# limuhit/360-Image-Compression

Hardware: AMD Instinct MI355X
Metric: ERP Mpixels/s enc+dec @512x1024 model-idx 3; bitstream bit-exact vs ref (higher is better)
Workload: dtype f32; 1 GPU; 192/GPU synthetic 512x1024 ERPs, model-idx 3 --ssim seed, latent+importance bitstreams, entropy enc+dec; streams=3, masks=smooth

## Files before the change

### 360-image-compression_amd/csrc/cconv4_kernels.hip

```cpp
#include "common.h"
#include "conv_plan.h"

#include "cconv_tree.h"
#include "need.h"

#define C4_COLS 68
#define C4_WSLOTS 128

static inline bool conv4_ok(const lic360_conv_plan *p) {
    return p->ksz == 5 && (p->cin == 1 || p->cin == 4) && p->cout >= 1 && p->cout <= 4 && p->ngroup <= 64;
}

__global__ void k_conv4_pack(const float *__restrict__ weight, float *__restrict__ quads, int wblk, int nb, int ngroup, int cin, int cout, int hidden) {
    const long per_net = (long)ngroup * ngroup * C4_WSLOTS * 4, total = per_net * nb;
    const int C = ngroup * cin, nout = ngroup * cout;
    for (long i = (long)blockIdx.x * blockDim.x + threadIdx.x; i < total; i += (long)gridDim.x * blockDim.x) {
        int r = (int)(i & 3), leaf = (int)((i >> 2) & 31), c = (int)((i >> 7) & 3);
        long t = i / (C4_WSLOTS * 4);
        int tc = (int)(t % ngroup), g = (int)((t / ngroup) % ngroup), b = (int)(t / ((long)ngroup * ngroup));
        int tap = cin == 4 ? leaf : c + 4 * leaf, gid = cin == 4 ? ((c - tap) & 3) : 0;
        float v = 0.0f;
        if (tap < 25 && r < cout) {
            int kh = tap / 5, kw = tap % 5;
            int L = g + 4 - kh - kw + hidden;
            if (L > ngroup) L = ngroup;
            if (tc < L) v = weight[(((long)b * nout + g * cout + r) * C + tc * cin + gid) * 25 + tap];
        }
        const long qb = (long)(b * ngroup + g) * wblk;
        const int ln = (leaf & 15) * 4 + r;
        if (cin == 4) quads[(qb + (tc >> 1)) * 1024 + c * 256 + ln * 4 + (tc & 1) * 2 + (leaf >> 4)] = v;
        else if (leaf < 16) quads[(qb + (tc >> 2)) * 1024 + c * 256 + ln * 4 + (tc & 3)] = v;
    }
}

LIC360_API int lic360_conv4_supported(const lic360_conv_plan *p) { return p && conv4_ok(p) ? 1 : 0; }
static inline long conv4_slot_floats(const lic360_conv_plan *p) { return (long)p->ngroup * p->ngroup * C4_WSLOTS * 4; }
static inline int conv4_wblk(const lic360_conv_plan *p) { return p->cin == 4 ? (p->ngroup + 1) / 2 : 2 * ((p->ngroup + 7) / 8); }
static inline long conv4_quad_floats(const lic360_conv_plan *p) { return (long)p->ngroup * conv4_wblk(p) * 1024; }
LIC360_API long lic360_conv4_packed_floats(const lic360_conv_plan *p) {
    return p && conv4_ok(p) ? conv4_quad_floats(p) : 0;
}
LIC360_API int lic360_conv4_pack(void *stream, const lic360_conv_plan *p, const float *weight, int nb, float *packed) {
    ARG_CHECK(p && conv4_ok(p) && weight && packed && nb > 0);
    const long total = conv4_slot_floats(p) * nb;
    HIP_TRY(hipMemsetAsync(packed, 0, (size_t)conv4_quad_floats(p) * nb * sizeof(float), (hipStream_t)stream));
    hipLaunchKernelGGL(k_conv4_pack, dim3(lic360_blocks(total, 4)), dim3(256), 0, (hipStream_t)stream, weight, packed, conv4_wblk(p), nb, p->ngroup,
                       p->cin, p->cout, p->constrain == 5 ? 0 : 1);
    LAUNCH_CHECK();
    return 0;
}

#define C4_PS 3
#define C4_THREADS (C4_PS * 4 * 64)
#define C4_COMB_FLOATS (C4_PS * 4 * 4 * 64)

#include "cconv4v6_dc.inc"

int lic360_cconv4_dc_plane_mode(void *stream, const lic360_conv_plan *p, const float *x, const float *packed4, const float *bias,
                                const float *act, const float *residual, float *out, int n, int h, int w, int nb, int psum, int x_mod, int mode) {
    ARG_CHECK(p && conv4_ok(p) && x && packed4 && bias && out && n > 0 && nb > 0 && n % nb == 0 && x_mod > 0 && x_mod <= n);
    if (psum < 0 || psum >= h + w + p->ngroup - 2) return 0;
    return launch_cconv4v6_dc((hipStream_t)stream, p, x, packed4, bias, act, residual, out, n, h, w, nb, psum, x_mod, (mode & 2) != 0,
                              (mode >> 2) & 3);
}
int lic360_cconv4_dc_plane_list(void *stream, const lic360_conv_plan *p, const float *x, const float *packed4, const float *bias,
                                const float *act, const float *residual, float *out, int n, int h, int w, int nb, int psum, int x_mod,
                                const void *list, const int *cnt, int cap) {
    ARG_CHECK(p && conv4_ok(p) && x && packed4 && bias && out && n > 0 && nb > 0 && n % nb == 0 && x_mod > 0 && x_mod <= n);
    if (psum < 0 || psum >= h + w + p->ngroup - 2) return 0;
    return launch_cconv4v6_dc_list((hipStream_t)stream, p, x, packed4, bias, act, residual, out, n, h, w, nb, psum, x_mod, (const uint4 *)list, cnt, cap);
}
int lic360_dc4_env_mode(void) {
    const char *gsm = getenv("LIC360_DC_GSTEP");
    return (getenv("LIC360_NOPACK") ? 2 : 0) | (gsm && gsm[0] == '1' ? 4 : (gsm && gsm[0] == '3' ? 8 : 0));
}
LIC360_API int lic360_cconv4_dc_plane(void *stream, const lic360_conv_plan *p, const float *x, const float *packed4, const float *bias,
                                      const float *act, const float *residual, float *out, int n, int h, int w, int nb, int psum, int x_mod) {
    static const int mode = lic360_dc4_env_mode();
    return lic360_cconv4_dc_plane_mode(stream, p, x, packed4, bias, act, residual, out, n, h, w, nb, psum, x_mod, mode);
}

#define C4_TAIL_FLOATS 4096
LIC360_API long lic360_conv4_buffer_floats(int layout, long planes, int h, int w) {
    if (planes <= 0 || h <= 0 || w <= 0 || layout != 0) return 0;
    return planes * ((long)D3_SP(h, w) * D3_HP(h)) + C4_TAIL_FLOATS;
}
LIC360_API int lic360_dc4_layout(int h, int w, int *rows, int *pitch, int *row0, int *col0) {
    ARG_CHECK(rows && pitch && row0 && col0 && h > 0 && w > 0);
    *rows = D3_SP(h, w); *pitch = D3_HP(h); *row0 = D3_S0; *col0 = D3_C0;
    return 0;
}
```

### 360-image-compression_amd/csrc/cconv4v6_dc.inc

```
#define D6_GRID 256
#define D6_TAPE_BLOCKS 16
#define D6_TAPE_WAVES 6
#define D3_S0 (4 + C4_PS - 1)
#define D3_C0 2
#define D3_SP(h, w) ((h) + (w) - 1 + 2 * D3_S0)
#define D3_HP(h) ((h) + 2 * D3_C0)
struct Dc3Args {
    const float *x, *packed, *bias, *act, *residual;
    float *out;
    int ngroup, cout, hidden, H, W, npb, x_mod, N, psum, n_gb, n_gbv, nseg, pack0, gstep;
    int wblk;
    int nprod;
    int tape_c, tape_n, tape_total;
    unsigned tape_magic;
    unsigned tape_nw4[2];
};
struct Dc3Packed {
    const float *x, *packed, *bias, *act, *residual;
    float *out;
    unsigned w0;
    unsigned hw;
    int npb, x_mod, N;
    unsigned pg;
    int wblk, tape_n, tape_total;
// ... 85 lines not shown
__device__ __forceinline__ void conv6_diags(f32x4 *acc, const float *r0, float w0, float w1) {
    static_for<9>([&](auto dd) {
        constexpr int d = decltype(dd)::value, kmin = d > 4 ? d - 4 : 0, kmax = d < 4 ? d : 4;
        if constexpr (d >= D_LO && d <= D_HI && (CIN == 4 || (d & 3) == CLS)) {
            static_for<kmax - kmin + 1>([&](auto kk) {
                constexpr int kh = kmin + decltype(kk)::value, tap = 5 * kh + (d - kh), i = CIN == 4 ? tap : (tap - CLS) / 4;
                acc[i] = mfma4<i % 16>(i < 16 ? w0 : w1, r0[d], acc[i]);
            });
        }
    });
    __builtin_amdgcn_sched_barrier(0);
}
template <int CIN, int CLS>
__device__ __forceinline__ void conv6_align(f32x4 *acc) {
    static_for<9>([&](auto dd) {
        constexpr int d = decltype(dd)::value, kmin = d > 4 ? d - 4 : 0, kmax = d < 4 ? d : 4;
        constexpr int k0 = kmax < 2 ? kmax : (kmin > 2 ? kmin : 2);
        if constexpr (CIN == 4 || (d & 3) == CLS) {
            static_for<kmax - kmin + 1>([&](auto kk) {
                constexpr int kh = kmin + decltype(kk)::value, tap = 5 * kh + (d - kh), i = CIN == 4 ? tap : (tap - CLS) / 4, sh = kh - k0;
                static_for<(sh > 0 ? sh : -sh)>([&](auto) {
#pragma unroll
                    for (int r = 0; r < 4; ++r) acc[i][r] = sh > 0 ? dpp_shl1(acc[i][r]) : dpp_shr1(acc[i][r]);
                });
            });
        }
    });
}

struct W8 {
    float a0, a1, a2, a3, b0, b1, b2, b3;
    template <int H, int J> __device__ __forceinline__ float get() const {
        if constexpr (H == 0) return J == 0 ? a0 : (J == 1 ? a1 : (J == 2 ? a2 : a3));
        else return J == 0 ? b0 : (J == 1 ? b1 : (J == 2 ? b2 : b3));
    }
};

#define D6_SEG_STEP 60
#define D6_NSEG(h) ((h) <= 64 ? 1 : 1 + ((h) - 62 + D6_SEG_STEP - 1) / D6_SEG_STEP)
#ifdef DC6_STAMP
__device__ unsigned long long dc6_stamps[256 * 12 * 10];
#ifndef DC6_STAMP_CIN
#define DC6_STAMP_CIN 4
#endif
#define DC6_T(i) do { if constexpr (CIN == DC6_STAMP_CIN && !SEG) { const unsigned long long t_ = __builtin_amdgcn_s_memtime(); st[i] += t_ - t0; t0 = t_; } } while (0)
LIC360_API int lic360_dc6_stamps(unsigned long long *host_out, int clear) {
    if (host_out) HIP_TRY(hipMemcpyFromSymbol(host_out, HIP_SYMBOL(dc6_stamps), sizeof(dc6_stamps)));
    if (clear) { static unsigned long long z[256 * 12 * 10]; HIP_TRY(hipMemcpyToSymbol(HIP_SYMBOL(dc6_stamps), z, sizeof(z))); }
    return 0;
}
#else
#define DC6_T(i)
#endif
template <int CIN, int CLS, bool SEG, bool LAT = false, bool TAPE = false, bool LIST = false>
__device__ __forceinline__ void dc6_body(const Dc3Args &a, const Dc3Tape *tape, const uint4 *__restrict__ list, const int *__restrict__ lcnt, float *xs, float *comb,
                                         int (*trec)[16], int tid, int lane, int ps) {
    static_assert(!LIST || (TAPE && !SEG && !LAT), "list launches are throughput-mode launches of images of at most 64 rows");
    constexpr int XQ = D6_XQ(CIN), XFL = D6_XFL(CIN);
    static_assert(XQ <= C4_THREADS, "one quad slot per thread");
    constexpr int XPLANE = D6_ROWS * D6_COLS;
    const int H = a.H, W = a.W, G = a.ngroup, S = H + W - 1, HP = D3_HP(H);
    const int gs = a.gstep;
    constexpr int TCS = CIN == 1 ? 4 : 1;
    const long SKP = (long)D3_SP(H, W) * HP, tcs = 4 * SKP;
    f32x4 acc[NAcc<CIN>::value];
#ifdef DC6_STAMP
    unsigned long long st[10] = {0, 0, 0, 0, 0, 0, 0, 0, 0, 0}, t0 = __builtin_amdgcn_s_memtime();
    const unsigned long long t_entry = t0;
#endif
    const bool flat = gs == 1;
    const int xcd = flat ? 0 : blockIdx.x & 7, xstep = flat ? 1 : 8, wg_in_xcd = flat ? blockIdx.x : blockIdx.x >> 3;
    const int wgs_per_xcd = flat ? D6_GRID : (D6_GRID - xcd + 7) >> 3;
    auto nth_task = [&](int k) __attribute__((always_inline)) { return k * wgs_per_xcd + ((k & 1) ? wgs_per_xcd - 1 - wg_in_xcd : wg_in_xcd); };
    const int ns_x = flat ? a.N : (a.N - xcd + 7) >> 3;
    const int nseg = SEG ? a.nseg : 1;
    constexpr bool PACK = true;
    const bool pack_last = PACK && SEG && a.pack0 != 0;
    const int per_j = SEG ? ns_x * (nseg - 1) + (pack_last ? (ns_x + 1) >> 1 : ns_x) : 0;
    const int tape_c = TAPE ? a.tape_c : 0;
    const unsigned nw4[2] = {a.tape_nw4[0], a.tape_nw4[1]};
    auto blk_tasks = [&](int j) __attribute__((always_inline)) {
        return tape_c ? a.tape_n * (int)((nw4[(j >> 3) & 1] >> ((j & 7) * 4)) & 15u) : ns_x;
    };
    uint4 lrec = make_uint4(0u, 0u, 0u, 0u);
    if constexpr (LIST) {
        if (CLS == 0 && ps == 0) {
            int u = nth_task(lane);
            if (u > a.tape_total - 1) u = a.tape_total - 1;
            lrec = list[(long)xcd * a.tape_total + u];
        }
    }
    int n_my_ = 0;
    if constexpr (LIST) n_my_ = __builtin_amdgcn_readfirstlane(lcnt[xcd]);
    else if constexpr (SEG) n_my_ = per_j * a.n_gbv;
    else if (tape_c) n_my_ = a.tape_total;
    else n_my_ = ns_x * a.n_gbv;
    const int n_my = n_my_;
    int pk = -1, pq = 0;
    auto decode = [&](int u, int &g0, int &n, int &s0, int &seg, int &nb2, int &prb, int &packed) __attribute__((always_inline)) {
        nb2 = -1; prb = 0; packed = 0;
        if constexpr (LIST) {
            uint4 r;
            if (pk < 64) {
                r.x = (unsigned)__builtin_amdgcn_readlane((int)lrec.x, pk); r.y = (unsigned)__builtin_amdgcn_readlane((int)lrec.y, pk);
                r.z = (unsigned)__builtin_amdgcn_readlane((int)lrec.z, pk); r.w = (unsigned)__builtin_amdgcn_readlane((int)lrec.w, pk);
            } else r = list[(long)xcd * a.tape_total + u];
            g0 = (int)(r.x & 127u);
            n = (int)(r.x >> 10);
            s0 = a.psum - g0;
            seg = 0;
            if ((r.x >> 7) & 7u) { seg = (int)(r.y & 0x3fffffu); nb2 = (int)r.z; prb = (int)r.w; packed = 4; }
            packed |= (int)((r.y >> 22) & 7u) << 4;
        } else if constexpr (!SEG) {
            int j = 0, rem = u;
            for (; j < a.n_gbv - 1 && rem >= blk_tasks(j); ++j) rem -= blk_tasks(j);
            g0 = (a.n_gb - 1 - j) * gs;
            s0 = a.psum - g0;
            seg = 0;
// ... 100 lines not shown
                }
                t_off = cov ? offA + sh : 0u;
                t_off0 = cov ? offA0 + sh : 0u;
            } else if (SEG && PACK && ipacked) {
                const bool hb = qc > 8;
                const unsigned shift = hb ? (unsigned)(((long)((inb >= 0 ? inb : n) % a.x_mod) - (long)(n % a.x_mod)) * G * CIN * SKP * 4 - 9 * 16) : 0u;
                t_off = offA + shift;
                t_off0 = offA0 + shift;
            } else {
                const int lo = is0 - (gs - 1) - W + 1 - irb, hi = (is0 < H - 1 ? is0 : H - 1) - irb;
                const bool col_ok = qc >= ((lo > 0 ? lo : 0) >> 2) && qc <= ((hi + 4) >> 2);
                t_off = col_ok ? offA : 0u;
                t_off0 = col_ok ? offA0 : 0u;
            }
        }
        const int gg = ig0 + ps < G ? ig0 + ps : G - 1;
        iwp = (const char *)(a.packed + (((long)(n / a.npb) * G + gg) * a.wblk) * 1024);
    };
    if (!ivalid) return;
    issue_setup();
    const long tcs_b = tcs * 4;
    constexpr int WPSTEP = CIN == 4 ? 4096 : 8192;
    const char *px = ixn, *pw = iwp;
    auto issue_x2 = [&](f32x4 &ra, f32x4 &rb, int &tc0) __attribute__((always_inline)) -> const char * {
        const char *pwr = pw;
        tc0 = itc;
        unsigned oa, ob;
        if constexpr (CIN == 4) {
            oa = rowA < irl - itc ? t_off : t_off0;
            ob = rowA < irl - itc - 1 ? t_off : t_off0;
        } else {
            const int ta = itc + tcoA, tb = ta + TCS;
            oa = rowA < irl - ta ? t_off : t_off0;
            ob = rowA < irl - tb ? t_off : t_off0;
            if (ta >= G) oa = offP0;
            if (tb >= G) ob = offP0;
        }
        ra = *(const f32x4 *)(px + oa);
        rb = *(const f32x4 *)(px + (itc + TCS < G ? tcs_b : 0) + ob);
        if (ivalid) {
            px += 2 * tcs_b;
            pw += WPSTEP;
            itc += 2 * TCS;
            if (itc >= iL) {
                itc = 0;
                ++iq;
                ivalid = rec(iq, 0) != 0;
                if (ivalid) { issue_setup(); px = ixn; pw = iwp; }
                else { px -= 2 * tcs_b; pw -= WPSTEP; itc = tc0; }
            }
        }
        return pwr;
    };
    auto issue_w2 = [&](const char *p, int tc0, W8 &w) __attribute__((always_inline)) {
        (void)tc0;
        const f32x4 v = *(const f32x4 *)(p + offW);
        w.a0 = v[0]; w.a1 = v[1];
        if constexpr (CIN == 4) { w.b0 = v[2]; w.b1 = v[3]; }
        else {
            const f32x4 u = *(const f32x4 *)(p + offW + 4096);
            w.a2 = v[2]; w.a3 = v[3];
            w.b0 = u[0]; w.b1 = u[1]; w.b2 = u[2]; w.b3 = u[3];
        }
    };
    constexpr bool MIDST = D6_STAGE_AT_END == 0 || CIN == 1 || LAT || LIST;
    constexpr int NB = D6_NB, NBUF = 2 * D6_NB;
    static_assert(NB == 1 || NB == 2, "one or two double steps per barrier");
    f32x4 xa0 = {0.f, 0.f, 0.f, 0.f}, xb0 = xa0, xa1 = xa0, xb1 = xa0;
    W8 w0, w1;
    int tcw;
    { const char *p = issue_x2(xa0, xb0, tcw); issue_w2(p, tcw, w0); }
    { const char *p = issue_x2(xa1, xb1, tcw); issue_w2(p, tcw, w1); }
    if (hasA) { *(f32x4 *)ldsA = xa0; *(f32x4 *)(ldsA + XFL) = xb0; }
    int tcw_next, tcw_next2 = 0;
    const char *pw_next = issue_x2(xa0, xb0, tcw_next), *pw_next2 = nullptr;
    if constexpr (NB == 2) {
        if (hasA) { *(f32x4 *)(ldsA + 2 * XFL) = xa1; *(f32x4 *)(ldsA + 3 * XFL) = xb1; }
        pw_next2 = issue_x2(xa1, xb1, tcw_next2);
    }
    const f32x4 zero4 = {0.f, 0.f, 0.f, 0.f};
    int tq = 0, tc = 0, g0 = 0, n = 0, Lwg = 0, g = 0, s = 0, step = 0;
    bool glive = false, lane_ok = false;
    int n_lane = 0;
    float e_bias = 0.f, e_act = 0.f, e_res = 0.f;
    long e_oi = 0;
    const float *const act_p = a.act ? a.act : a.bias, *const res_p = a.residual ? a.residual : a.x;
    const float *const xl0 = xs + (C4_PS - 1 - ps) * D6_COLS + lane;
    auto task_setup = [&]() __attribute__((always_inline)) {
        g0 = rec(tq, 1); n = rec(tq, 2);
        const int s0 = rec(tq, 3), seg = rec(tq, 4), nb2 = rec(tq, 5), prb = rec(tq, 6);
        const int pk7 = rec(tq, 7), packed = pk7 & 15;
        Lwg = steps_of(g0);
        g = g0 + ps;
        s = s0 - ps;
        const int rb = packed == 4 ? 0 : ((SEG && !packed) ? D6_SEG_STEP * seg : prb);
        int row = rb + lane;
        n_lane = n;
        bool half_ok = true;
        if (TAPE && packed == 4) {
            half_ok = false;
            row = 0;
#pragma unroll
            for (int wi = 0; wi < 3; ++wi) {
                const unsigned wd = (unsigned)(wi == 0 ? seg : (wi == 1 ? nb2 : prb));
                const int k = wd & 7, slo = (wd >> 3) & 63, shi = (wd >> 9) & 63, a0 = (wd >> 15) & 63;
                if ((wd >> 21) != 0 && lane >= a0 && lane <= a0 + (shi - slo)) { half_ok = true; row = slo + lane - a0; n_lane = n + 8 * k; }
            }
        } else if (SEG && PACK && packed) {
            if (lane >= 36) { row = rb + lane - 36; n_lane = nb2 >= 0 ? nb2 : n; half_ok = nb2 >= 0; }
            else half_ok = lane < 28;
        }
        int sc;
        {
            int lo = s >= W ? s - W + 1 : 0, hi = s < H ? s : H - 1;
            const int segx = packed == 4 ? 0 : seg;
            if (lo < seg_lo(segx)) lo = seg_lo(segx);
            if (hi > seg_hi(segx)) hi = seg_hi(segx);
            glive = g < G && ps < gs && s >= 0 && s < S && lo <= hi && ((pk7 >> (4 + ps)) & 1) != 0;
            lane_ok = glive && half_ok && row >= lo && row <= hi;
            sc = s < 0 ? 0 : (s >= S ? S - 1 : s);
        }
#pragma unroll
        for (int i = 0; i < NAcc<CIN>::value; ++i) acc[i] = zero4;
        tc = 0;
        const int nout = G * a.cout, gc = g < G ? g : G - 1;
        const int o = gc * a.cout + (CLS < a.cout ? CLS : a.cout - 1), bid = (n / a.npb) * nout + o;
        e_oi = ((long)n_lane * nout + o) * SKP + (long)(sc + D3_S0) * HP + row + D3_C0;
        e_bias = a.bias[bid];
        e_act = act_p[bid];
        e_res = res_p[a.residual ? e_oi : 0];
    };
    auto epilogue = [&]() __attribute__((always_inline)) {
        conv6_align<CIN, CLS>(acc);
        const f32x4 part = tree4_eval<CIN, CLS>(acc);
        float *const cb = CIN == 1 ? comb + (tq & 1) * C4_COMB_FLOATS : comb;
#pragma unroll
        for (int r = 0; r < 4; ++r) cb[((ps * 4 + CLS) * 4 + r) * 64 + lane] = part[r];
        __syncthreads();
        const int r = CLS;
        if (lane_ok && r < a.cout) {
            const float f0 = cb[((ps * 4 + 0) * 4 + r) * 64 + lane], f1 = cb[((ps * 4 + 1) * 4 + r) * 64 + lane];
            const float f2 = cb[((ps * 4 + 2) * 4 + r) * 64 + lane], f3 = cb[((ps * 4 + 3) * 4 + r) * 64 + lane];
            float sv = ((f0 + f2) + (f1 + f3)) + e_bias;
            if (a.act) { if (sv < 0) sv = sv * e_act; }
            if (a.residual) sv = sv + e_res;
            a.out[e_oi] = sv;
        }
    };
    task_setup();
#define DC6_SUB(H_, J_, W_)                                                                     \
    if constexpr ((J_) < TCS) {                                                                 \
        constexpr int k = (H_) * TCS + (J_);                                                    \
        const int dl = dlim - k;                     \
        if (dl > 0 && tc + k < Lwg) {                                                           \
            float r0[9];                                                                        \
            conv6_load<CIN, CLS, XPLANE>(r0, xl + (H_) * XFL + (J_) * XPLANE);                  \
            __builtin_amdgcn_sched_barrier(0);                                                  \
            const float wa = W_.template get<(H_), (CIN == 4 ? 0 : (J_))>(), wb = W_.template get<(H_), 1>(); \
            conv6_diags<CIN, CLS, 0, 3>(acc, r0, wa, wb);                                       \
            if (dl > 4) conv6_diags<CIN, CLS, 4, 5>(acc, r0, wa, wb);                           \
            if (dl > 6) conv6_diags<CIN, CLS, 6, 8>(acc, r0, wa, wb);                           \
        }                                                                                       \
    }
#define DC6_HALF(H_, W_) DC6_SUB(H_, 0, W_) DC6_SUB(H_, 1, W_) DC6_SUB(H_, 2, W_) DC6_SUB(H_, 3, W_)
#define D6_STAGE_WRITE(XA_, XB_)                                                                \
        if (hasA) {                                                                             \
            float *q = ldsA + ((step + NB) & (NBUF - 1)) * (2 * XFL);                           \
            *(f32x4 *)q = XA_;                                                                  \
            *(f32x4 *)(q + XFL) = XB_;                                                          \
        }
#define D6_STAGE_BLOCK(XA_, XB_)                                                                \
        D6_STAGE_WRITE(XA_, XB_)                                                                \
        DC6_T(8);                        \
        pw_new = issue_x2(XA_, XB_, tcw_new);                                                   \
        __builtin_amdgcn_sched_barrier(0);
#define D6_STAGE_MID(XA_, XB_) if constexpr (MIDST) { D6_STAGE_BLOCK(XA_, XB_) }
#define D6_STAGE_END(XA_, XB_) if constexpr (!MIDST) { D6_STAGE_BLOCK(XA_, XB_) }
#define DC6_SUBSTEP(XA_, XB_, W_)                                                               \
    {                                                                                           \
        if (tc >= Lwg) {                                                                        \
            epilogue();                                                                         \
            ++tq;                                                                               \
            if (producer) produce();               \
            if (rec(tq, 0)) task_setup();                                                       \
            else { done = true; glive = false; Lwg = 0x7fffffff; }                              \
            DC6_ST7                                                                             \
        }                                                                                       \
        DC6_T(0);                                                                               \
        if (NB == 1 || (step & 1) == 0) __syncthreads();                                        \
        DC6_T(1);                                                                               \
        const int dlim = glive ? g + 4 + a.hidden - tc : 0;                                     \
        const float *xl = xl0 + (step & (NBUF - 1)) * (2 * XFL);                                \
        int tcw_new = 0;                                                                        \
        const char *pw_new = nullptr;                                                           \
        DC6_HALF(0, W_)                                                                         \
        DC6_T(2);                                                                               \
        D6_STAGE_MID(XA_, XB_)                                                                  \
        DC6_T(3);                                                                               \
        DC6_HALF(1, W_)                                                                         \
        D6_STAGE_END(XA_, XB_)                                                                  \
        DC6_T(4);                                                                               \
        issue_w2(pw_next, tcw_next, W_);                                                        \
        if constexpr (NB == 2) { pw_next = pw_next2; tcw_next = tcw_next2; pw_next2 = pw_new; tcw_next2 = tcw_new; } \
        else { pw_next = pw_new; tcw_next = tcw_new; }                                          \
        tc += 2 * TCS;                                                                          \
        ++step;                                                                                 \
        DC6_T(5);                                                                               \
        DC6_ST6                                                                                 \
    }
#ifdef DC6_STAMP
#define DC6_ST6 st[6] += 1;
#define DC6_ST7 st[7] += 1;
#else
#define DC6_ST6
#define DC6_ST7
#endif
    bool done = false;
    do {
        if constexpr (NB == 2) {
            DC6_SUBSTEP(xa0, xb0, w0)
            DC6_SUBSTEP(xa1, xb1, w1)
        } else {
            DC6_SUBSTEP(xa1, xb1, w0)
            DC6_SUBSTEP(xa0, xb0, w1)
        }
    } while (!done);
#ifdef DC6_STAMP
    if constexpr (CIN == DC6_STAMP_CIN && !SEG) {
        st[9] = __builtin_amdgcn_s_memtime() - t_entry;
        if (lane == 0) for (int i = 0; i < 10; ++i) dc6_stamps[((blockIdx.x & 255) * 12 + ps * 4 + CLS) * 10 + i] += st[i];
    }
#endif
#undef DC6_ST6
#undef DC6_ST7
#undef DC6_HALF
#undef DC6_SUB
#undef DC6_SUBSTEP
}

template <int CIN, bool SEG, bool LAT, bool TAPE, bool LIST = false>
__device__ __forceinline__ void dc6_kernel(const Dc3Packed &p, const Dc3Tape *tape, const uint4 *list = nullptr, const int *lcnt = nullptr) {
    __shared__ float xs[4 * D6_NB * D6_XFL(CIN)];
    __shared__ float comb[2 * C4_COMB_FLOATS];
    __shared__ int trec[8][16];
    const Dc3Args a = dc6_unpack(p);
    const int tid = threadIdx.x, lane = tid & 63;
    const int wave = __builtin_amdgcn_readfirstlane(tid >> 6), ps = wave >> 2, cls = wave & 3;
    switch (cls) {
        case 0: dc6_body<CIN, 0, SEG, LAT, TAPE, LIST>(a, tape, list, lcnt, xs, comb, trec, tid, lane, ps); break;
        case 1: dc6_body<CIN, 1, SEG, LAT, TAPE, LIST>(a, tape, list, lcnt, xs, comb, trec, tid, lane, ps); break;
        case 2: dc6_body<CIN, 2, SEG, LAT, TAPE, LIST>(a, tape, list, lcnt, xs, comb, trec, tid, lane, ps); break;
        default: dc6_body<CIN, 3, SEG, LAT, TAPE, LIST>(a, tape, list, lcnt, xs, comb, trec, tid, lane, ps); break;
    }
}
template <int CIN, bool SEG, bool LAT = false>
__global__ __launch_bounds__(C4_THREADS) void k_cconv4v6(Dc3Packed p) { dc6_kernel<CIN, SEG, LAT, false>(p, nullptr); }
template <int CIN>
__global__ __launch_bounds__(C4_THREADS) void k_cconv4v6t(Dc3Packed p, Dc3Tape tape) { dc6_kernel<CIN, false, false, true>(p, &tape); }
template <int CIN>
__global__ __launch_bounds__(C4_THREADS) void k_cconv4v6l(Dc3Packed p, const uint4 *list, const int *lcnt) { dc6_kernel<CIN, false, false, true, true>(p, nullptr, list, lcnt); }

static void dc6_build_tape(Dc3Args &a, Dc3Tape &tape, int h, int w, int cin, int n, int gs, bool nopack) {
    a.tape_c = 0; a.tape_n = 1; a.tape_total = 0; a.tape_magic = 0u; a.tape_nw4[0] = a.tape_nw4[1] = 0u;
    for (int j = 0; j < D6_TAPE_BLOCKS; ++j) tape.s[j] = 0u;
    const int S = h + w - 1, m = a.npb / 8;
    int c = 0;
    for (int t = D6_TAPE_WAVES; t >= 2 && !c; --t) if (m % t == 0) c = t;
    const bool ok = !nopack && a.nseg == 1 && gs == C4_PS && n % 8 == 0 && a.npb % 8 == 0 && c >= 2 && a.x_mod % (8 * c) == 0 && a.n_gbv <= D6_TAPE_BLOCKS &&
                    8.0 * c * a.ngroup * cin * (double)D3_SP(h, w) * D3_HP(h) * 4.0 < 4294967296.0;
    if (!ok) return;
    long old_tasks = 0, new_tasks = 0;
    int nws[D6_TAPE_BLOCKS];
    for (int j = 0; j < a.n_gbv; ++j) {
        const int gb = a.n_gb - 1 - j, s0 = a.psum - gb * C4_PS;
        int lo = 1 << 30, hi = -1;
        for (int q = 0; q < C4_PS; ++q) {
            const int sq = s0 - q;
            if (gb * C4_PS + q >= a.ngroup || sq < 0 || sq >= S) continue;
            const int l = sq >= w ? sq - w + 1 : 0, u = sq < h ? sq : h - 1;
            if (l < lo) lo = l;
            if (u > hi) hi = u;
        }
        int nw = 0, k = 0, slo = lo;
        unsigned starts = 0u;
        bool fits = hi >= 0;
        while (fits && k < c) {
            if (nw >= D6_TAPE_WAVES) { fits = false; break; }
            if (nw & 1) starts |= ((unsigned)k | (unsigned)slo << 3) << (9 * (nw >> 1));
            unsigned pc[3];
            if (dc6_wave_pieces(lo, hi, h, c, k, slo, pc) == 0) fits = false;
            ++nw;
        }
        if (!fits || nw >= c) {
            nw = c;
            starts = 0u;
        }
        tape.s[j] = starts;
        a.tape_nw4[j >> 3] |= (unsigned)nw << ((j & 7) * 4);
        nws[j] = nw;
        new_tasks += (long)nw * (m / c);
        old_tasks += m;
    }
    if (new_tasks > 0 && new_tasks < old_tasks) {
        a.tape_c = c;
        a.tape_n = n / 8 / c;
        a.tape_magic = (unsigned)((4294967296ull + a.tape_n - 1) / a.tape_n);
        for (int j = 0; j < a.n_gbv; ++j) a.tape_total += a.tape_n * nws[j];
    }
}

static bool dc6_schedule(Dc3Args &a, Dc3Tape &tape, int ngroup, int cin, int cout, int constrain, int n, int h, int w, int nb, int psum, int x_mod, bool nopack, int gstep_mode) {
    a.ngroup = ngroup; a.cout = cout; a.hidden = constrain == 5 ? 0 : 1; a.H = h; a.W = w; a.npb = n / nb; a.x_mod = x_mod; a.N = n;
    a.psum = psum;
    const int S = h + w - 1;
    int gb_lo = 1 << 30, gb_hi = -1;
    const int n_gb3 = (ngroup + C4_PS - 1) / C4_PS;
    const int gs = gstep_mode == 1 || (gstep_mode == 0 && (long)n * n_gb3 <= 128 && D6_NSEG(h) == 1) ? 1 : C4_PS;
    a.gstep = gs;
    {
        const int tcs2 = cin == 4 ? 2 : 8, lmin0 = (gs - 1) + 4 + a.hidden, lmin = lmin0 < ngroup ? lmin0 : ngroup;
        const int dmin = (lmin + tcs2 - 1) / tcs2, lead = (4 + dmin - 1) / dmin;
        a.nprod = lead + 2 < 6 ? lead + 2 : 6;
    }
    const int n_gb_all = (ngroup + gs - 1) / gs;
    for (int gb = 0; gb < n_gb_all; ++gb) {
        int s0 = psum - gb * gs;
        if (s0 - (gs - 1) >= S || s0 < 0) continue;
        if (gb < gb_lo) gb_lo = gb;
        if (gb > gb_hi) gb_hi = gb;
    }
    a.tape_c = 0; a.pack0 = 0;
    if (gb_hi < 0) return false;
    a.n_gb = gb_hi + 1;
    a.n_gbv = gb_hi - gb_lo + 1;
    a.nseg = D6_NSEG(h);
    dc6_build_tape(a, tape, h, w, cin, n, gs, nopack);
    if (a.nseg > 1 && a.npb % 16 == 0 && x_mod % 16 == 0 && !nopack && gs == C4_PS && h >= 28 && D6_SEG_STEP * (a.nseg - 1) + 2 >= h - 28 + 2) a.pack0 = 1;
    return true;
}

static int launch_cconv4v6_dc(hipStream_t stream, const lic360_conv_plan *p, const float *x, const float *packed4, const float *bias,
                              const float *act, const float *residual, float *out, int n, int h, int w, int nb, int psum, int x_mod, bool nopack,
                              int gstep_mode) {
    Dc3Args a;
    a.x = x; a.packed = packed4; a.wblk = conv4_wblk(p); a.bias = bias; a.act = act; a.residual = residual; a.out = out;
    ARG_CHECK(16.0 * p->ngroup * p->cin * (double)D3_SP(h, w) * D3_HP(h) * 4.0 < 4294967296.0);
    ARG_CHECK(h < 32768 && w < 32768 && D6_NSEG(h) <= 15 && p->ngroup <= 127 && p->cout <= 7 && psum >= 0 && psum < 65536);
    Dc3Tape tape;
    if (!dc6_schedule(a, tape, p->ngroup, p->cin, p->cout, p->constrain, n, h, w, nb, psum, x_mod, nopack, gstep_mode)) return 0;
    const int gs = a.gstep;
    const Dc3Packed pk = dc6_pack(a);
    if (a.nseg > 1) {
        if (p->cin == 4) hipLaunchKernelGGL((k_cconv4v6<4, true>), dim3(D6_GRID), dim3(C4_THREADS), 0, stream, pk);
        else hipLaunchKernelGGL((k_cconv4v6<1, true>), dim3(D6_GRID), dim3(C4_THREADS), 0, stream, pk);
    } else if (a.tape_c) {
        if (p->cin == 4) hipLaunchKernelGGL((k_cconv4v6t<4>), dim3(D6_GRID), dim3(C4_THREADS), 0, stream, pk, tape);
        else hipLaunchKernelGGL((k_cconv4v6t<1>), dim3(D6_GRID), dim3(C4_THREADS), 0, stream, pk, tape);
    } else if (p->cin == 4 && gs == 1) hipLaunchKernelGGL((k_cconv4v6<4, false, true>), dim3(D6_GRID), dim3(C4_THREADS), 0, stream, pk);
    else if (p->cin == 4) hipLaunchKernelGGL((k_cconv4v6<4, false>), dim3(D6_GRID), dim3(C4_THREADS), 0, stream, pk);
    else hipLaunchKernelGGL((k_cconv4v6<1, false>), dim3(D6_GRID), dim3(C4_THREADS), 0, stream, pk);
    LAUNCH_CHECK();
    return 0;
}

static int launch_cconv4v6_dc_list(hipStream_t stream, const lic360_conv_plan *p, const float *x, const float *packed4, const float *bias,
                                   const float *act, const float *residual, float *out, int n, int h, int w, int nb, int psum, int x_mod,
                                   const uint4 *list, const int *lcnt, int cap) {
    Dc3Args a;
    a.x = x; a.packed = packed4; a.wblk = conv4_wblk(p); a.bias = bias; a.act = act; a.residual = residual; a.out = out;
    ARG_CHECK(64.0 * p->ngroup * p->cin * (double)D3_SP(h, w) * D3_HP(h) * 4.0 < 4294967296.0);
    ARG_CHECK(h <= 64 && w < 32768 && p->ngroup <= 127 && p->cout <= 7 && psum >= 0 && psum < 65536 && p->cin == 4 && list && lcnt && cap > 0);
    ARG_CHECK(n % 8 == 0 && (n / nb) % 8 == 0 && x_mod == n);
    Dc3Tape tape;
    if (!dc6_schedule(a, tape, p->ngroup, p->cin, p->cout, p->constrain, n, h, w, nb, psum, x_mod, true, 3)) return 0;
    ARG_CHECK(a.gstep == C4_PS && a.nseg == 1);
    a.tape_c = 1;
    a.tape_total = cap;
    const Dc3Packed pk = dc6_pack(a);
    hipLaunchKernelGGL((k_cconv4v6l<4>), dim3(D6_GRID), dim3(C4_THREADS), 0, stream, pk, list, lcnt);
    LAUNCH_CHECK();
    return 0;
}

LIC360_API int lic360_dc4_tape_layout(int ngroup, int cin, int n, int nb, int h, int w, int psum, int x_mod, int *tape_c, int *n_blocks, int *blocks, int *nwaves, unsigned *windows) {
    ARG_CHECK(tape_c && n_blocks && blocks && nwaves && windows && ngroup > 0 && ngroup <= 64 && (cin == 1 || cin == 4) && n > 0 && nb > 0 && n % nb == 0 && h > 0 && w > 0 && x_mod > 0);
    Dc3Args a;
    *tape_c = 0; *n_blocks = 0;
    Dc3Tape tape;
    if (!dc6_schedule(a, tape, ngroup, cin, 4, cin == 4 ? 6 : 5, n, h, w, nb, psum, x_mod, false, 0)) return 0;
    *n_blocks = a.n_gbv < 24 ? a.n_gbv : 24;
    *tape_c = a.tape_c;
    for (int j = 0; j < 24 * 6 * 3; ++j) windows[j] = 0u;
    for (int j = 0; j < a.n_gbv && j < 24; ++j) {
        blocks[j] = (a.n_gb - 1 - j) * a.gstep;
        nwaves[j] = a.tape_c ? (int)((a.tape_nw4[(j >> 3) & 1] >> ((j & 7) * 4)) & 15u) : 0;
        if (!a.tape_c || nwaves[j] >= a.tape_c) continue;
        int lo = 1 << 30, hi = -1;
        for (int q = 0; q < C4_PS; ++q) {
            const int sq = psum - blocks[j] - q;
            if (blocks[j] + q >= ngroup || sq < 0 || sq >= h + w - 1) continue;
            const int l = sq >= w ? sq - w + 1 : 0, u = sq < h ? sq : h - 1;
            if (l < lo) lo = l;
            if (u > hi) hi = u;
        }
        for (int t = 0; t < nwaves[j]; ++t) {
            int k, slo;
            dc6_wave_start(tape.s[j], lo, hi, h, a.tape_c, t, k, slo);
            dc6_wave_pieces(lo, hi, h, a.tape_c, k, slo, &windows[(j * 6 + t) * 3]);
        }
    }
    return 0;
}
```

### 360-image-compression_amd/csrc/codec_fused.hip

```cpp
#include "common.h"
#include "conv_plan.h"
#include "ac_core.h"
#include "lic360_exact_math.h"
#include "gmm_tables.h"
#include "need.h"
#include <vector>
#include <cstring>
#include <algorithm>
#include <thread>
#include <atomic>
#include <memory>
#include <type_traits>
#include <immintrin.h>

struct AcDevState {
    uint32_t low, high, code;
    int nacc, error, pad;
    long pos;
    unsigned long long acc;
};
struct DcLayout {
    int rows, pitch, row0, col0;
    __host__ __device__ long plane() const { return (long)rows * pitch; }
    __host__ __device__ long cell(int th, int tw) const { return (long)(th + tw + row0) * pitch + th + col0; }
// ... 1476 lines not shown
    if (out) {
        HIP_TRY(hipDeviceSynchronize());
        HIP_TRY(hipMemcpy(out, c->stats, 2 * NEED_LAYERS * NEED_STAT_G * sizeof(unsigned long long), hipMemcpyDeviceToHost));
        HIP_TRY(hipMemset(c->stats, 0, 2 * NEED_LAYERS * NEED_STAT_G * sizeof(unsigned long long)));
    }
    return 0;
}
__global__ void k_fill_enc(float *buf, long planes, int H, int W, int hp, int wp, int off, float v) {
    GRID_STRIDE(i, planes * H * W) {
        const int x = (int)(i % W), y = (int)((i / W) % H);
        buf[(i / ((long)H * W)) * hp * wp + e_cell(y, x, wp, off)] = v;
    }
}
__global__ void k_fill_dec(float *buf, long planes, int H, int W, DcLayout sk, float v) {
    GRID_STRIDE(i, planes * H * W) {
        const int x = (int)(i % W), y = (int)((i / W) % H);
        buf[(i / ((long)H * W)) * sk.plane() + sk.cell(y, x)] = v;
    }
}
LIC360_API int lic360_codec_debug_fill(void *stream, lic360_codec *c, float value) {
    ARG_CHECK(c && value == value && value - value == 0.0f);
    hipStream_t s = (hipStream_t)stream;
    const long B = c->maxB, G = c->G;
    for (int i = 0; i < 3; ++i) {
        hipLaunchKernelGGL(k_fill_enc, dim3(lic360_blocks(3 * B * 4 * G * c->HW, 4)), dim3(256), 0, s, c->e_buf[i], 3 * B * 4 * G, c->H, c->W, c->e_hp, c->e_wp, c->e_off, value);
        LAUNCH_CHECK();
    }
    for (int i = 0; i < 11; ++i) {
        hipLaunchKernelGGL(k_fill_dec, dim3(lic360_blocks(3 * B * 4 * G * c->HW, 4)), dim3(256), 0, s, c->d_act[i], 3 * B * 4 * G, c->H, c->W, c->sk, value);
        LAUNCH_CHECK();
    }
    hipLaunchKernelGGL(k_fill_dec, dim3(lic360_blocks(3 * B * 3 * G * c->HW, 4)), dim3(256), 0, s, c->d_y, 3 * B * 3 * G, c->H, c->W, c->sk, value);
    LAUNCH_CHECK();
    return 0;
}
LIC360_API int lic360_codec_debug_lists(lic360_codec *c, int which, void *host_out, long bytes, int *cap_out) {
    ARG_CHECK(c && host_out && bytes >= 0 && which >= 0 && which <= 4 && c->skip);
    HIP_TRY(hipDeviceSynchronize());
    const void *src = nullptr;
    long have = 0;
    if (which == 0) { src = c->need; have = (long)c->maxB * NEED_LAYERS * c->HW; }
    else if (which == 1) { src = c->ecl.cnt; have = NEED_LAYERS * 8 * 4L; }
    else if (which == 2) { src = c->ecl.list; have = (long)NEED_LAYERS * 8 * c->ecl.cap * 4; }
    else if (which == 3) { src = c->dcl.cnt; have = c->dcl.list ? (long)NEED_LAYERS * c->P * 8 * 4 : 0; }
    else { src = c->dcl.list; have = c->dcl.list ? (long)NEED_LAYERS * c->P * 8 * c->dcl.cap * 16 : 0; }
    if (cap_out) *cap_out = which <= 2 ? c->ecl.cap : c->dcl.cap;
    ARG_CHECK(src && bytes <= have);
    HIP_TRY(hipMemcpy(host_out, src, (size_t)bytes, hipMemcpyDeviceToHost));
    return 0;
}

LIC360_API const char *lic360_codec_kernel_names(void) {
    return "ec_first=k_cconv16<1, false>;ec_hidden=k_cconv16s+k_cconv16<4, false>;ec_last=k_cconv16<4, true>;"
           "dc_first=k_cconv4v6<1, false, false>+k_cconv4v6t<1>;"
           "dc_hidden=k_cconv4v6l<4>+k_cconv4v6t<4>+k_cconv4v6<4, false, false>+k_cconv4v6<4, false, true>;"
           "dc_last=k_cconv4v6l<4>+k_cconv4v6t<4>+k_cconv4v6<4, false, false>+k_cconv4v6<4, false, true>;"
           "imp_ec=k_cconv144<1, false, 2>;imp_dc=k_cconv144<1, true, 2>+k_cconv144<1, true, 1>";
}
```

Measured before the change: 60.59 Mpixel/s.

## Process three nets per task in first decoder conv layer to share input loads

Adds a NETS template parameter so the first decode layer (cin=1, nb=3, throughput mode) has each task compute all three networks' outputs from one shared input tile, keeping three accumulator sets and loading per-net weights in halves. The schedule is redone over n/nb images with a single net-block, which cuts the number of input staging and LDS passes by up to three times. In exchange it raises register pressure from tripled accumulators and weights, can lower occupancy, and adds one barrier per net in the epilogue. An environment flag can turn it off.

```diff
diff --git a/360-image-compression_amd/csrc/cconv4_kernels.hip b/360-image-compression_amd/csrc/cconv4_kernels.hip
--- a/360-image-compression_amd/csrc/cconv4_kernels.hip
+++ b/360-image-compression_amd/csrc/cconv4_kernels.hip
@@ -61,7 +61,7 @@
     ARG_CHECK(p && conv4_ok(p) && x && packed4 && bias && out && n > 0 && nb > 0 && n % nb == 0 && x_mod > 0 && x_mod <= n);
     if (psum < 0 || psum >= h + w + p->ngroup - 2) return 0;
     return launch_cconv4v6_dc((hipStream_t)stream, p, x, packed4, bias, act, residual, out, n, h, w, nb, psum, x_mod, (mode & 2) != 0,
-                              (mode >> 2) & 3);
+                              (mode >> 2) & 3, (mode & 16) != 0);
 }
 int lic360_cconv4_dc_plane_list(void *stream, const lic360_conv_plan *p, const float *x, const float *packed4, const float *bias,
                                 const float *act, const float *residual, float *out, int n, int h, int w, int nb, int psum, int x_mod,
@@ -72,7 +72,7 @@
 }
 int lic360_dc4_env_mode(void) {
     const char *gsm = getenv("LIC360_DC_GSTEP");
-    return (getenv("LIC360_NOPACK") ? 2 : 0) | (gsm && gsm[0] == '1' ? 4 : (gsm && gsm[0] == '3' ? 8 : 0));
+    return (getenv("LIC360_NOPACK") ? 2 : 0) | (gsm && gsm[0] == '1' ? 4 : (gsm && gsm[0] == '3' ? 8 : 0)) | (getenv("LIC360_DC_NONETS") ? 16 : 0);
 }
 LIC360_API int lic360_cconv4_dc_plane(void *stream, const lic360_conv_plan *p, const float *x, const float *packed4, const float *bias,
                                       const float *act, const float *residual, float *out, int n, int h, int w, int nb, int psum, int x_mod) {
diff --git a/360-image-compression_amd/csrc/cconv4v6_dc.inc b/360-image-compression_amd/csrc/cconv4v6_dc.inc
--- a/360-image-compression_amd/csrc/cconv4v6_dc.inc
+++ b/360-image-compression_amd/csrc/cconv4v6_dc.inc
@@ -161,10 +161,12 @@
 #else
 #define DC6_T(i)
 #endif
-template <int CIN, int CLS, bool SEG, bool LAT = false, bool TAPE = false, bool LIST = false>
+template <int CIN, int CLS, bool SEG, bool LAT = false, bool TAPE = false, bool LIST = false, int NETS = 1>
 __device__ __forceinline__ void dc6_body(const Dc3Args &a, const Dc3Tape *tape, const uint4 *__restrict__ list, const int *__restrict__ lcnt, float *xs, float *comb,
                                          int (*trec)[16], int tid, int lane, int ps) {
     static_assert(!LIST || (TAPE && !SEG && !LAT), "list launches are throughput-mode launches of images of at most 64 rows");
+    static_assert(NETS == 1 || (NETS == 3 && CIN == 1 && !SEG && !LAT && !LIST), "three nets per task: the first layer in throughput mode");
+    constexpr int NA = NAcc<CIN>::value;
     constexpr int XQ = D6_XQ(CIN), XFL = D6_XFL(CIN);
     static_assert(XQ <= C4_THREADS, "one quad slot per thread");
     constexpr int XPLANE = D6_ROWS * D6_COLS;
@@ -172,7 +174,7 @@
     const int gs = a.gstep;
     constexpr int TCS = CIN == 1 ? 4 : 1;
     const long SKP = (long)D3_SP(H, W) * HP, tcs = 4 * SKP;
-    f32x4 acc[NAcc<CIN>::value];
+    f32x4 acc[NETS * NA];
 #ifdef DC6_STAMP
     unsigned long long st[10] = {0, 0, 0, 0, 0, 0, 0, 0, 0, 0}, t0 = __builtin_amdgcn_s_memtime();
     const unsigned long long t_entry = t0;
@@ -379,25 +381,41 @@
         }
         return pwr;
     };
-    auto issue_w2 = [&](const char *p, int tc0, W8 &w) __attribute__((always_inline)) {
+    const long wnet_b = NETS > 1 ? (long)G * a.wblk * 4096 : 0;
+    auto issue_w2 = [&](const char *p, int tc0, W8 *ws) __attribute__((always_inline)) {
         (void)tc0;
-        const f32x4 v = *(const f32x4 *)(p + offW);
-        w.a0 = v[0]; w.a1 = v[1];
-        if constexpr (CIN == 4) { w.b0 = v[2]; w.b1 = v[3]; }
-        else {
-            const f32x4 u = *(const f32x4 *)(p + offW + 4096);
-            w.a2 = v[2]; w.a3 = v[3];
-            w.b0 = u[0]; w.b1 = u[1]; w.b2 = u[2]; w.b3 = u[3];
+#pragma unroll
+        for (int net = 0; net < NETS; ++net) {
+            W8 &w = ws[net];
+            const f32x4 v = *(const f32x4 *)(p + net * wnet_b + offW);
+            w.a0 = v[0]; w.a1 = v[1];
+            if constexpr (CIN == 4) { w.b0 = v[2]; w.b1 = v[3]; }
+            else {
+                const f32x4 u = *(const f32x4 *)(p + net * wnet_b + offW + 4096);
+                w.a2 = v[2]; w.a3 = v[3];
+                w.b0 = u[0]; w.b1 = u[1]; w.b2 = u[2]; w.b3 = u[3];
+            }
+        }
+    };
+    auto issue_wh = [&](const char *p, auto hh, W8 *ws) __attribute__((always_inline)) {
+        constexpr int hf = decltype(hh)::value;
+#pragma unroll
+        for (int net = 0; net < NETS; ++net) {
+            W8 &w = ws[net];
+            const f32x4 v = *(const f32x4 *)(p + net * wnet_b + offW + hf * 4096);
+            if constexpr (hf == 0) { w.a0 = v[0]; w.a1 = v[1]; w.a2 = v[2]; w.a3 = v[3]; }
+            else { w.b0 = v[0]; w.b1 = v[1]; w.b2 = v[2]; w.b3 = v[3]; }
         }
     };
     constexpr bool MIDST = D6_STAGE_AT_END == 0 || CIN == 1 || LAT || LIST;
     constexpr int NB = D6_NB, NBUF = 2 * D6_NB;
     static_assert(NB == 1 || NB == 2, "one or two double steps per barrier");
     f32x4 xa0 = {0.f, 0.f, 0.f, 0.f}, xb0 = xa0, xa1 = xa0, xb1 = xa0;
-    W8 w0, w1;
+    W8 w0[NETS], w1[NETS];
+    const char *pw_one = nullptr;
     int tcw;
     { const char *p = issue_x2(xa0, xb0, tcw); issue_w2(p, tcw, w0); }
-    { const char *p = issue_x2(xa1, xb1, tcw); issue_w2(p, tcw, w1); }
+    { const char *p = issue_x2(xa1, xb1, tcw); if constexpr (NETS == 1) issue_w2(p, tcw, w1); else pw_one = p; }
     if (hasA) { *(f32x4 *)ldsA = xa0; *(f32x4 *)(ldsA + XFL) = xb0; }
     int tcw_next, tcw_next2 = 0;
     const char *pw_next = issue_x2(xa0, xb0, tcw_next), *pw_next2 = nullptr;
@@ -409,7 +427,7 @@
     int tq = 0, tc = 0, g0 = 0, n = 0, Lwg = 0, g = 0, s = 0, step = 0;
     bool glive = false, lane_ok = false;
     int n_lane = 0;
-    float e_bias = 0.f, e_act = 0.f, e_res = 0.f;
+    float e_bias[NETS], e_act[NETS], e_res = 0.f;
     long e_oi = 0;
     const float *const act_p = a.act ? a.act : a.bias, *const res_p = a.residual ? a.residual : a.x;
     const float *const xl0 = xs + (C4_PS - 1 - ps) * D6_COLS + lane;
@@ -448,31 +466,36 @@
             sc = s < 0 ? 0 : (s >= S ? S - 1 : s);
         }
 #pragma unroll
-        for (int i = 0; i < NAcc<CIN>::value; ++i) acc[i] = zero4;
+        for (int i = 0; i < NETS * NA; ++i) acc[i] = zero4;
         tc = 0;
         const int nout = G * a.cout, gc = g < G ? g : G - 1;
         const int o = gc * a.cout + (CLS < a.cout ? CLS : a.cout - 1), bid = (n / a.npb) * nout + o;
         e_oi = ((long)n_lane * nout + o) * SKP + (long)(sc + D3_S0) * HP + row + D3_C0;
-        e_bias = a.bias[bid];
-        e_act = act_p[bid];
+#pragma unroll
+        for (int net = 0; net < NETS; ++net) { e_bias[net] = a.bias[bid + net * nout]; e_act[net] = act_p[bid + net * nout]; }
         e_res = res_p[a.residual ? e_oi : 0];
     };
     auto epilogue = [&]() __attribute__((always_inline)) {
-        conv6_align<CIN, CLS>(acc);
-        const f32x4 part = tree4_eval<CIN, CLS>(acc);
-        float *const cb = CIN == 1 ? comb + (tq & 1) * C4_COMB_FLOATS : comb;
-#pragma unroll
-        for (int r = 0; r < 4; ++r) cb[((ps * 4 + CLS) * 4 + r) * 64 + lane] = part[r];
-        __syncthreads();
-        const int r = CLS;
-        if (lane_ok && r < a.cout) {
-            const float f0 = cb[((ps * 4 + 0) * 4 + r) * 64 + lane], f1 = cb[((ps * 4 + 1) * 4 + r) * 64 + lane];
-            const float f2 = cb[((ps * 4 + 2) * 4 + r) * 64 + lane], f3 = cb[((ps * 4 + 3) * 4 + r) * 64 + lane];
-            float sv = ((f0 + f2) + (f1 + f3)) + e_bias;
-            if (a.act) { if (sv < 0) sv = sv * e_act; }
-            if (a.residual) sv = sv + e_res;
-            a.out[e_oi] = sv;
-        }
+        static_for<NETS>([&](auto nn) {
+            constexpr int net = decltype(nn)::value;
+            f32x4 *const ac = acc + net * NA;
+            conv6_align<CIN, CLS>(ac);
+            const f32x4 part = tree4_eval<CIN, CLS>(ac);
+            float *const cb = NETS > 1 ? comb + net * C4_COMB_FLOATS : (CIN == 1 ? comb + (tq & 1) * C4_COMB_FLOATS : comb);
+#pragma unroll
+            for (int r = 0; r < 4; ++r) cb[((ps * 4 + CLS) * 4 + r) * 64 + lane] = part[r];
+            __syncthreads();
+            const int r = CLS;
+            if (lane_ok && r < a.cout) {
+                const long oi = NETS > 1 ? e_oi + net * ((long)a.npb * G * a.cout * SKP) : e_oi;
+                const float f0 = cb[((ps * 4 + 0) * 4 + r) * 64 + lane], f1 = cb[((ps * 4 + 1) * 4 + r) * 64 + lane];
+                const float f2 = cb[((ps * 4 + 2) * 4 + r) * 64 + lane], f3 = cb[((ps * 4 + 3) * 4 + r) * 64 + lane];
+                float sv = ((f0 + f2) + (f1 + f3)) + e_bias[net];
+                if (a.act) { if (sv < 0) sv = sv * e_act[net]; }
+                if (a.residual) sv = sv + (NETS > 1 ? a.residual[oi] : e_res);
+                a.out[oi] = sv;
+            }
+        });
     };
     task_setup();
 #define DC6_SUB(H_, J_, W_)                                                                     \
@@ -483,10 +506,13 @@
             float r0[9];                                                                        \
             conv6_load<CIN, CLS, XPLANE>(r0, xl + (H_) * XFL + (J_) * XPLANE);                  \
             __builtin_amdgcn_sched_barrier(0);                                                  \
-            const float wa = W_.template get<(H_), (CIN == 4 ? 0 : (J_))>(), wb = W_.template get<(H_), 1>(); \
-            conv6_diags<CIN, CLS, 0, 3>(acc, r0, wa, wb);                                       \
-            if (dl > 4) conv6_diags<CIN, CLS, 4, 5>(acc, r0, wa, wb);                           \
-            if (dl > 6) conv6_diags<CIN, CLS, 6, 8>(acc, r0, wa, wb);                           \
+            static_for<NETS>([&](auto nn) {          \
+                constexpr int net = decltype(nn)::value;                                        \
+                const float wa = W_[net].template get<(H_), (CIN == 4 ? 0 : (J_))>(), wb = W_[net].template get<(H_), 1>(); \
+                conv6_diags<CIN, CLS, 0, 3>(acc + net * NA, r0, wa, wb);                        \
+                if (dl > 4) conv6_diags<CIN, CLS, 4, 5>(acc + net * NA, r0, wa, wb);            \
+                if (dl > 6) conv6_diags<CIN, CLS, 6, 8>(acc + net * NA, r0, wa, wb);            \
+            });                                                                                 \
         }                                                                                       \
     }
 #define DC6_HALF(H_, W_) DC6_SUB(H_, 0, W_) DC6_SUB(H_, 1, W_) DC6_SUB(H_, 2, W_) DC6_SUB(H_, 3, W_)
@@ -521,13 +547,15 @@
         int tcw_new = 0;                                                                        \
         const char *pw_new = nullptr;                                                           \
         DC6_HALF(0, W_)                                                                         \
+        if constexpr (NETS > 1) issue_wh(pw_one, IC<0>{}, W_);                                  \
         DC6_T(2);                                                                               \
         D6_STAGE_MID(XA_, XB_)                                                                  \
         DC6_T(3);                                                                               \
         DC6_HALF(1, W_)                                                                         \
         D6_STAGE_END(XA_, XB_)                                                                  \
         DC6_T(4);                                                                               \
-        issue_w2(pw_next, tcw_next, W_);                                                        \
+        if constexpr (NETS > 1) { issue_wh(pw_one, IC<1>{}, W_); pw_one = pw_next; }            \
+        else issue_w2(pw_next, tcw_next, W_);                                                   \
         if constexpr (NB == 2) { pw_next = pw_next2; tcw_next = tcw_next2; pw_next2 = pw_new; tcw_next2 = tcw_new; } \
         else { pw_next = pw_new; tcw_next = tcw_new; }                                          \
         tc += 2 * TCS;                                                                          \
@@ -545,8 +573,13 @@
     bool done = false;
     do {
         if constexpr (NB == 2) {
-            DC6_SUBSTEP(xa0, xb0, w0)
-            DC6_SUBSTEP(xa1, xb1, w1)
+            if constexpr (NETS == 1) {
+                DC6_SUBSTEP(xa0, xb0, w0)
+                DC6_SUBSTEP(xa1, xb1, w1)
+            } else {
+                DC6_SUBSTEP(xa0, xb0, w0)
+                DC6_SUBSTEP(xa1, xb1, w0)
+            }
         } else {
             DC6_SUBSTEP(xa1, xb1, w0)
             DC6_SUBSTEP(xa0, xb0, w1)
@@ -565,25 +598,25 @@
 #undef DC6_SUBSTEP
 }
 
-template <int CIN, bool SEG, bool LAT, bool TAPE, bool LIST = false>
+template <int CIN, bool SEG, bool LAT, bool TAPE, bool LIST = false, int NETS = 1>
 __device__ __forceinline__ void dc6_kernel(const Dc3Packed &p, const Dc3Tape *tape, const uint4 *list = nullptr, const int *lcnt = nullptr) {
     __shared__ float xs[4 * D6_NB * D6_XFL(CIN)];
-    __shared__ float comb[2 * C4_COMB_FLOATS];
+    __shared__ float comb[(NETS > 1 ? NETS : 2) * C4_COMB_FLOATS];
     __shared__ int trec[8][16];
     const Dc3Args a = dc6_unpack(p);
     const int tid = threadIdx.x, lane = tid & 63;
     const int wave = __builtin_amdgcn_readfirstlane(tid >> 6), ps = wave >> 2, cls = wave & 3;
     switch (cls) {
-        case 0: dc6_body<CIN, 0, SEG, LAT, TAPE, LIST>(a, tape, list, lcnt, xs, comb, trec, tid, lane, ps); break;
-        case 1: dc6_body<CIN, 1, SEG, LAT, TAPE, LIST>(a, tape, list, lcnt, xs, comb, trec, tid, lane, ps); break;
-        case 2: dc6_body<CIN, 2, SEG, LAT, TAPE, LIST>(a, tape, list, lcnt, xs, comb, trec, tid, lane, ps); break;
-        default: dc6_body<CIN, 3, SEG, LAT, TAPE, LIST>(a, tape, list, lcnt, xs, comb, trec, tid, lane, ps); break;
-    }
-}
-template <int CIN, bool SEG, bool LAT = false>
-__global__ __launch_bounds__(C4_THREADS) void k_cconv4v6(Dc3Packed p) { dc6_kernel<CIN, SEG, LAT, false>(p, nullptr); }
-template <int CIN>
-__global__ __launch_bounds__(C4_THREADS) void k_cconv4v6t(Dc3Packed p, Dc3Tape tape) { dc6_kernel<CIN, false, false, true>(p, &tape); }
+        case 0: dc6_body<CIN, 0, SEG, LAT, TAPE, LIST, NETS>(a, tape, list, lcnt, xs, comb, trec, tid, lane, ps); break;
+        case 1: dc6_body<CIN, 1, SEG, LAT, TAPE, LIST, NETS>(a, tape, list, lcnt, xs, comb, trec, tid, lane, ps); break;
+        case 2: dc6_body<CIN, 2, SEG, LAT, TAPE, LIST, NETS>(a, tape, list, lcnt, xs, comb, trec, tid, lane, ps); break;
+        default: dc6_body<CIN, 3, SEG, LAT, TAPE, LIST, NETS>(a, tape, list, lcnt, xs, comb, trec, tid, lane, ps); break;
+    }
+}
+template <int CIN, bool SEG, bool LAT = false, int NETS = 1>
+__global__ __launch_bounds__(C4_THREADS) void k_cconv4v6(Dc3Packed p) { dc6_kernel<CIN, SEG, LAT, false, false, NETS>(p, nullptr); }
+template <int CIN, int NETS = 1>
+__global__ __launch_bounds__(C4_THREADS) void k_cconv4v6t(Dc3Packed p, Dc3Tape tape) { dc6_kernel<CIN, false, false, true, false, NETS>(p, &tape); }
 template <int CIN>
 __global__ __launch_bounds__(C4_THREADS) void k_cconv4v6l(Dc3Packed p, const uint4 *list, const int *lcnt) { dc6_kernel<CIN, false, false, true, true>(p, nullptr, list, lcnt); }
 
@@ -666,18 +699,31 @@
     return true;
 }
 
+static bool dc6_schedule_nets(Dc3Args &a, Dc3Tape &tape, int ngroup, int cin, int cout, int constrain, int n, int h, int w, int nb, int psum, int x_mod, bool nopack,
+                              int gstep_mode, bool no_nets, int *nets) {
+    *nets = 1;
+    if (!dc6_schedule(a, tape, ngroup, cin, cout, constrain, n, h, w, nb, psum, x_mod, nopack, gstep_mode)) return false;
+    if (no_nets || cin != 1 || nb != 3 || (long)x_mod * nb != n || a.gstep != C4_PS || a.nseg != 1) return true;
+    *nets = 3;
+    return dc6_schedule(a, tape, ngroup, cin, cout, constrain, n / nb, h, w, 1, psum, x_mod, nopack, 3);
+}
+
 static int launch_cconv4v6_dc(hipStream_t stream, const lic360_conv_plan *p, const float *x, const float *packed4, const float *bias,
                               const float *act, const float *residual, float *out, int n, int h, int w, int nb, int psum, int x_mod, bool nopack,
-                              int gstep_mode) {
+                              int gstep_mode, bool no_nets) {
     Dc3Args a;
     a.x = x; a.packed = packed4; a.wblk = conv4_wblk(p); a.bias = bias; a.act = act; a.residual = residual; a.out = out;
     ARG_CHECK(16.0 * p->ngroup * p->cin * (double)D3_SP(h, w) * D3_HP(h) * 4.0 < 4294967296.0);
     ARG_CHECK(h < 32768 && w < 32768 && D6_NSEG(h) <= 15 && p->ngroup <= 127 && p->cout <= 7 && psum >= 0 && psum < 65536);
     Dc3Tape tape;
-    if (!dc6_schedule(a, tape, p->ngroup, p->cin, p->cout, p->constrain, n, h, w, nb, psum, x_mod, nopack, gstep_mode)) return 0;
+    int nets;
+    if (!dc6_schedule_nets(a, tape, p->ngroup, p->cin, p->cout, p->constrain, n, h, w, nb, psum, x_mod, nopack, gstep_mode, no_nets, &nets)) return 0;
     const int gs = a.gstep;
     const Dc3Packed pk = dc6_pack(a);
-    if (a.nseg > 1) {
+    if (nets == 3) {
+        if (a.tape_c) hipLaunchKernelGGL((k_cconv4v6t<1, 3>), dim3(D6_GRID), dim3(C4_THREADS), 0, stream, pk, tape);
+        else hipLaunchKernelGGL((k_cconv4v6<1, false, false, 3>), dim3(D6_GRID), dim3(C4_THREADS), 0, stream, pk);
+    } else if (a.nseg > 1) {
         if (p->cin == 4) hipLaunchKernelGGL((k_cconv4v6<4, true>), dim3(D6_GRID), dim3(C4_THREADS), 0, stream, pk);
         else hipLaunchKernelGGL((k_cconv4v6<1, true>), dim3(D6_GRID), dim3(C4_THREADS), 0, stream, pk);
     } else if (a.tape_c) {
@@ -714,7 +760,8 @@
     Dc3Args a;
     *tape_c = 0; *n_blocks = 0;
     Dc3Tape tape;
-    if (!dc6_schedule(a, tape, ngroup, cin, 4, cin == 4 ? 6 : 5, n, h, w, nb, psum, x_mod, false, 0)) return 0;
+    int nets;
+    if (!dc6_schedule_nets(a, tape, ngroup, cin, 4, cin == 4 ? 6 : 5, n, h, w, nb, psum, x_mod, false, 0, false, &nets)) return 0;
     *n_blocks = a.n_gbv < 24 ? a.n_gbv : 24;
     *tape_c = a.tape_c;
     for (int j = 0; j < 24 * 6 * 3; ++j) windows[j] = 0u;
diff --git a/360-image-compression_amd/csrc/codec_fused.hip b/360-image-compression_amd/csrc/codec_fused.hip
--- a/360-image-compression_amd/csrc/codec_fused.hip
+++ b/360-image-compression_amd/csrc/codec_fused.hip
@@ -1552,8 +1552,8 @@
 
 LIC360_API const char *lic360_codec_kernel_names(void) {
     return "ec_first=k_cconv16<1, false>;ec_hidden=k_cconv16s+k_cconv16<4, false>;ec_last=k_cconv16<4, true>;"
-           "dc_first=k_cconv4v6<1, false, false>+k_cconv4v6t<1>;"
-           "dc_hidden=k_cconv4v6l<4>+k_cconv4v6t<4>+k_cconv4v6<4, false, false>+k_cconv4v6<4, false, true>;"
-           "dc_last=k_cconv4v6l<4>+k_cconv4v6t<4>+k_cconv4v6<4, false, false>+k_cconv4v6<4, false, true>;"
+           "dc_first=k_cconv4v6t<1, 3>+k_cconv4v6<1, false, false, 3>+k_cconv4v6<1, false, false, 1>;"
+           "dc_hidden=k_cconv4v6l<4>+k_cconv4v6t<4, 1>+k_cconv4v6<4, false, false, 1>+k_cconv4v6<4, false, true, 1>;"
+           "dc_last=k_cconv4v6l<4>+k_cconv4v6t<4, 1>+k_cconv4v6<4, false, false, 1>+k_cconv4v6<4, false, true, 1>;"
            "imp_ec=k_cconv144<1, false, 2>;imp_dc=k_cconv144<1, true, 2>+k_cconv144<1, true, 1>";
 }
```

Measured after the change: 61.33 Mpixel/s (median of 6 runs). 1.2% higher.
